# ChikaYan/mvs_gaussian_splatting

Hardware: AMD Instinct MI355X
Metric: Mpixels/s fwd + train-step ms @1080p, 6M Gaussians, 1->8 MI355X (higher is better)
Workload: dtype f32

## Files before the change

### mvs_gaussian_splatting_amd/csrc/gsr_api.hip

```cpp
#include <hip/hip_runtime.h>
#include <dlfcn.h>
#include <stdio.h>
#include <string.h>
#include <atomic>
#include <mutex>
#include <string>
#include <vector>

#include "gsr_common.h"
#include "gsr_launch.h"

using namespace gsr;

namespace {
thread_local std::string g_err = "";

int fail(int code, const char* msg) {
  g_err = msg;
  return code;
}
int hip_fail(hipError_t e, const char* where) {
  g_err = std::string(where) + ": " + hipGetErrorString(e);
  return (int)e;
}
// ... 157 lines not shown

size_t gsr_geom_bytes(int32_t P) { return GeomLayout(P < 0 ? 0 : P).bytes; }
size_t gsr_image_bytes(int32_t width, int32_t height) { return ImageLayout(width, height).bytes; }
size_t gsr_binning_bytes(uint32_t num_rendered, uint32_t num_visible, int32_t, int32_t, int32_t mode) {
  return BinLayout(num_rendered, num_visible, mode).bytes;
}
size_t gsr_backward_bytes(int32_t P, uint32_t num_rendered) { return BwdLayout(P, num_rendered).bytes; }
size_t gsr_camera_grad_bytes(int32_t P) { return camera_grad_bytes(P); }
size_t gsr_sort_scratch_bytes(uint32_t n) { return SortLayout(n).bytes; }

}

static void enqueue_depth_top_pass(const GsrParams* p, void* geom_ws, hipStream_t s);

enum TopPass { TOP_PASS_WITH, TOP_PASS_LATER, TOP_PASS_NEVER };
static int enqueue_stage1(const GsrParams* p, void* geom_ws, int32_t* radii, hipStream_t s, uint32_t capacity,
                          hipEvent_t counted, TopPass top_pass) {
  const GeomLayout L(p->P);
  {
    StageTimer t(p, GSR_STAGE_PREPROCESS_FWD, s);
    launch_preprocess_fwd(*p, at<GeomRec>(geom_ws, L.rec), at<BinInfo>(geom_ws, L.bin),
                          at<uint32_t>(geom_ws, L.block_sums), at<uint32_t>(geom_ws, L.block_vis), radii,
                          at<uint32_t>(geom_ws, L.block_big), at<uint32_t>(geom_ws, L.big_list),
                          at<uint2>(geom_ws, L.block_range), s);
  }
  if (int rc = check(p, s, "preprocess_fwd")) return rc;
  uint32_t* total = at<uint32_t>(geom_ws, L.total);
  {
    StageTimer t(p, GSR_STAGE_SCAN, s);
    launch_scan_block_sums(at<uint32_t>(geom_ws, L.block_sums), at<uint32_t>(geom_ws, L.block_offs), total + TOTAL_R,
                           at<uint32_t>(geom_ws, L.block_vis), at<uint32_t>(geom_ws, L.block_vis_offs), total + TOTAL_V,
                           L.nblocks, s, p->counts_pinned, at<uint2>(geom_ws, L.block_range),
                           at<uint32_t>(geom_ws, L.block_big), at<uint32_t>(geom_ws, L.block_big_offs), total + TOTAL_BIG);
  }
  if (int rc = check(p, s, "scan_block_sums")) return rc;
  if (counted) GSR_HIP(hipEventRecord(counted, s));
  if (p->binning_mode != GSR_BINNING_KEYS64) {
    StageTimer t(p, GSR_STAGE_SORT, s);
    launch_compact_visible(p->P, at<BinInfo>(geom_ws, L.bin), at<uint32_t>(geom_ws, L.block_vis_offs),
                           at<uint32_t>(geom_ws, L.block_offs),
                           p->forward_only ? nullptr : at<uint32_t>(geom_ws, L.slot_base), total, capacity,
                           (p->width + TILE - 1) / TILE, at<uint32_t>(geom_ws, L.dkey_a), at<uint2>(geom_ws, L.didx_a), s,
                           top_pass != TOP_PASS_NEVER);
    launch_sort_pairs_u32_v64(at<uint32_t>(geom_ws, L.dkey_a), at<uint2>(geom_ws, L.didx_a),
                              at<uint32_t>(geom_ws, L.dkey_b), at<uint2>(geom_ws, L.didx_b), (uint32_t)p->P,
                              DEPTH_SORT_BITS, at<char>(geom_ws, L.dsort), s, total + TOTAL_V);
    if (top_pass == TOP_PASS_WITH) enqueue_depth_top_pass(p, geom_ws, s);
// ... 274 lines not shown
  const ImageLayout I(p->width, p->height);
  GradRow* rows = at<GradRow>(bwd_ws, Wl.rows);
  uint8_t* flags = at<uint8_t>(bwd_ws, Wl.flags);
  const GeomRec* rec = at<GeomRec>(geom_ws, L.rec);
  if (R > 0) {
    if (!bin_ws) return fail(GSR_E_BADARG, "bin_ws is NULL");
    const SortedViews sv = sorted_views(bin_ws, R, V, p->width, p->height, p->binning_mode);
    const uint32_t* point_list = sv.point_list;
    GSR_HIP(hipMemsetAsync(flags, 0, R, s));
    {
      StageTimer t(p, GSR_STAGE_RENDER_BWD, s);
      launch_render_bwd(p->width, p->height, at<uint2>(img_ws, I.ranges), point_list, rec,
                        at<uint32_t>(geom_ws, L.slot_base), p->bg,
                        at<float>(img_ws, I.final_T), at<uint32_t>(img_ws, I.n_contrib),
                        at<uint32_t>(img_ws, I.tile_max), dL_dout_color, rows, flags,
                        at<uint32_t>(img_ws, I.tile_order), s, sv.inst_mask);
    }
    if (int rc = check(p, s, "render_bwd")) return rc;
  }
  {
    StageTimer t(p, GSR_STAGE_PREPROCESS_BWD, s);
    launch_sum_big_rows(at<uint32_t>(geom_ws, L.total) + TOTAL_BIG, at<uint32_t>(geom_ws, L.block_big_offs), L.nblocks,
                        at<uint32_t>(geom_ws, L.big_list), rec, at<uint32_t>(geom_ws, L.slot_base), rows, flags, s);
    launch_preprocess_bwd(*p, radii, rec, at<uint32_t>(geom_ws, L.slot_base), rows, flags, *grads, s);
  }
  return check(p, s, "preprocess_bwd");
}

int gsr_profile_create(void** handle) {
  if (!handle) return fail(GSR_E_BADARG, "handle is NULL");
  *handle = new Profile();
  return 0;
}
int gsr_profile_destroy(void* handle) {
  Profile* pr = static_cast<Profile*>(handle);
  if (!pr) return 0;
  for (auto& sp : pr->used) { if (sp.a) (void)hipEventDestroy(sp.a); if (sp.b) (void)hipEventDestroy(sp.b); }
  for (auto e : pr->pool) (void)hipEventDestroy(e);
  delete pr;
  return 0;
}
int gsr_profile_collect(void* handle, double* ms_sum, uint32_t* counts) {
  Profile* pr = static_cast<Profile*>(handle);
  if (!pr || !ms_sum || !counts) return fail(GSR_E_BADARG, "NULL argument");
  std::vector<Profile::Span> spans;
  {
    std::lock_guard<std::mutex> lock(pr->mu);
// ... 542 lines not shown
```

### mvs_gaussian_splatting_amd/csrc/gsr_common.h

```cpp
#pragma once
#include <hip/hip_runtime.h>
#include <stdint.h>
#include "../../include/gsr.h"

namespace gsr {

constexpr int TILE = 16;
constexpr int WAVE = 64;
constexpr float NEAR_Z = 0.2f;
constexpr float DILATION = 0.3f;
constexpr float FOV_GUARD = 1.3f;
constexpr float ALPHA_MAX = 0.99f;
constexpr float ALPHA_MIN = 1.0f / 255.0f;
constexpr float T_STOP = 0.0001f;

struct __attribute__((aligned(64))) GeomRec {
  float x, y, cxx, cxy;
  float cyy, opacity, r, g;
  float b, ext_x, ext_y;
  uint32_t tile_mask;
  uint32_t rect_min;
  uint32_t rect_wh;
  float kk;
  float isyy;
// ... 66 lines not shown
#ifndef GSR_SORT_ITEMS
#define GSR_SORT_ITEMS 8
#endif
constexpr int SORT_ITEMS = GSR_SORT_ITEMS;
constexpr int SORT_TILE = SORT_THREADS * SORT_ITEMS;
constexpr int RADIX_BITS = 9;
constexpr int RADIX = 1 << RADIX_BITS;

struct SortLayout {
  size_t hist, totals, totals_odd, bytes;
  uint32_t nblocks;
  __host__ __device__ explicit SortLayout(uint32_t n) {
    nblocks = (n + SORT_TILE - 1) / SORT_TILE;
    if (nblocks == 0) nblocks = 1;
    nblocks += RADIX;
    size_t o = 0;
    hist = o;   o = align_up(o + 4 * (size_t)RADIX * nblocks, 256);
    totals = o; o = align_up(o + 4 * (size_t)RADIX, 256);
    totals_odd = o; o = align_up(o + 4 * (size_t)RADIX, 256);
    bytes = o;
  }
};

struct GeomLayout {
  size_t rec, bin, offsets, slot_base, block_sums, block_offs, block_vis, block_vis_offs, block_range, total;
  size_t dkey_a, dkey_b, didx_a, didx_b, dsort, big_list, block_big, block_big_offs, bytes;
  int nblocks;
  __host__ __device__ explicit GeomLayout(int P) {
    nblocks = (P + PRE_BLOCK - 1) / PRE_BLOCK;
    size_t o = 0;
    rec = o;        o = align_up(o + sizeof(GeomRec) * (size_t)P, 256);
    bin = o;        o = align_up(o + sizeof(BinInfo) * (size_t)P, 256);
    offsets = o;    o = align_up(o + 4 * (size_t)P, 256);
    slot_base = o;  o = align_up(o + 4 * (size_t)P, 256);
    block_sums = o; o = align_up(o + 4 * (size_t)(nblocks + 1), 256);
    block_offs = o; o = align_up(o + 4 * (size_t)(nblocks + 1), 256);
    block_vis = o;  o = align_up(o + 4 * (size_t)(nblocks + 1), 256);
    block_vis_offs = o; o = align_up(o + 4 * (size_t)(nblocks + 1), 256);
    block_range = o; o = align_up(o + 8 * (size_t)(nblocks + 1), 256);
    total = o;      o = align_up(o + 64, 256);
    dkey_a = o;     o = align_up(o + 4 * (size_t)P, 256);
    dkey_b = o;     o = align_up(o + 4 * (size_t)P, 256);
    didx_a = o;     o = align_up(o + 8 * (size_t)P, 256);
    didx_b = o;     o = align_up(o + 8 * (size_t)P, 256);
    dsort = o;      o = align_up(o + SortLayout((uint32_t)(P > 0 ? P : 1)).bytes, 256);
    big_list = o;   o = align_up(o + 4 * (size_t)nblocks * PRE_BLOCK, 256);
    block_big = o;  o = align_up(o + 4 * (size_t)(nblocks + 1), 256);
    block_big_offs = o; o = align_up(o + 4 * (size_t)(nblocks + 1), 256);
    bytes = o;
  }
};

enum {
  TOTAL_R = 0,
  TOTAL_V = 1,
  TOTAL_BIG = 2,
  TOTAL_DEPTH_INV_MIN = 4,
  TOTAL_DEPTH_MAX = 5,
  TOTAL_TOP_PASS_N = 6,
  TOTAL_R_CLAMPED = 7
};
constexpr int DEPTH_SORT_BITS = 24;

struct ImageLayout {
  size_t final_T, n_contrib, ranges, tile_max, tile_order, bytes;
  int grid_x, grid_y, tiles;
  __host__ __device__ ImageLayout(int W, int H) {
    grid_x = (W + TILE - 1) / TILE;
    grid_y = (H + TILE - 1) / TILE;
    tiles = grid_x * grid_y;
    size_t o = 0;
// ... 99 lines not shown
```

### mvs_gaussian_splatting_amd/csrc/gsr_launch.h

```cpp
#pragma once
#include "gsr_common.h"

namespace gsr {

void launch_preprocess_fwd(const GsrParams& p, GeomRec* rec, BinInfo* bin, uint32_t* block_sums, uint32_t* block_vis,
                           int32_t* radii, uint32_t* block_big, uint32_t* big_list, uint2* block_range, hipStream_t s);
void launch_sum_big_rows(const uint32_t* big_count, const uint32_t* big_offs, int nb, const uint32_t* big_list,
                         const GeomRec* rec, const uint32_t* slot_base, GradRow* rows, uint8_t* row_flags, hipStream_t s);
void launch_scan_block_sums(const uint32_t* sums_a, uint32_t* offs_a, uint32_t* total_a, const uint32_t* sums_b,
                            uint32_t* offs_b, uint32_t* total_b, int nb, hipStream_t s,
                            uint32_t* host_mirror = nullptr, const uint2* block_range = nullptr,
                            const uint32_t* sums_c = nullptr, uint32_t* offs_c = nullptr, uint32_t* total_c = nullptr);
void launch_preprocess_bwd(const GsrParams& p, const int32_t* radii, const GeomRec* rec, const uint32_t* slot_base,
                           const GradRow* rows,
                           const uint8_t* row_flags, const GsrGrads& g, hipStream_t s);
size_t camera_grad_bytes(int P);
void launch_camera_grad_finish(const GsrGrads& g, int nslots, hipStream_t s);

void launch_duplicate_with_keys(int P, int grid_x, const BinInfo* bin, const uint32_t* block_offs, uint32_t* slot_base,
                                uint32_t* point_offsets, uint64_t* keys, uint32_t* vals, hipStream_t s);
bool launch_sort_pairs(uint64_t* keys_a, uint32_t* vals_a, uint64_t* keys_b, uint32_t* vals_b, uint32_t n,
                       int end_bit, void* scratch, hipStream_t s);
struct SortedRuns {
  uint2* runs_rel;
  uint32_t n_keys;
  bool valid;
  bool relative;
  const uint32_t* totals_last;
  int lo_bits, hi_bits;
};
bool launch_sort_pairs_u32(uint32_t* keys_a, uint32_t* vals_a, uint32_t* keys_b, uint32_t* vals_b, uint32_t n,
                           int end_bit, void* scratch, hipStream_t s, const uint32_t* n_dev = nullptr,
                           SortedRuns* runs = nullptr);
void launch_identify_tile_ranges_u32(uint32_t R, const uint32_t* tiles, uint2* ranges, hipStream_t s,
                                     const uint32_t* r_dev = nullptr);
inline int sort_passes(int end_bit) { return (end_bit + RADIX_BITS - 1) / RADIX_BITS; }
void launch_identify_tile_ranges(uint32_t R, const uint64_t* keys, uint2* ranges, hipStream_t s);
void launch_build_tile_order(int tiles, const uint2* ranges, uint32_t* order, hipStream_t s);
// ... 117 lines not shown
```

### mvs_gaussian_splatting_amd/csrc/preprocess.hip

```cpp
#include "gsr_common.h"
#include "gsr_launch.h"

namespace gsr {

constexpr float SH_C0 = 0.28209479177387814f;
constexpr float SH_C1 = 0.4886025119029199f;
constexpr float SH_C2_0 = 1.0925484305920792f;
constexpr float SH_C2_1 = -1.0925484305920792f;
constexpr float SH_C2_2 = 0.31539156525252005f;
constexpr float SH_C2_3 = -1.0925484305920792f;
constexpr float SH_C2_4 = 0.5462742152960396f;
constexpr float SH_C3_0 = -0.5900435899266435f;
constexpr float SH_C3_1 = 2.890611442640554f;
constexpr float SH_C3_2 = -0.4570457994644658f;
constexpr float SH_C3_3 = 0.3731763325901154f;
constexpr float SH_C3_4 = -0.4570457994644658f;
constexpr float SH_C3_5 = 1.445305721320277f;
constexpr float SH_C3_6 = -0.5900435899266435f;

struct Mat4 { float m[16]; };

__device__ inline void load_mat(const float* __restrict__ src, Mat4& d) {
#pragma unroll
  for (int i = 0; i < 16; ++i) d.m[i] = src[i];
}
// ... 56 lines not shown
#pragma unroll
  for (int ch = 0; ch < 3; ++ch) {
    float res = SH_C0 * sh(0, ch);
    if (deg > 0) {
      res = res - SH_C1 * y * sh(1, ch) + SH_C1 * z * sh(2, ch) - SH_C1 * x * sh(3, ch);
      if (deg > 1) {
        const float xx = x * x, yy = y * y, zz = z * z, xy = x * y, yz = y * z, xz = x * z;
        res = res + SH_C2_0 * xy * sh(4, ch) + SH_C2_1 * yz * sh(5, ch) +
              SH_C2_2 * (2.0f * zz - xx - yy) * sh(6, ch) + SH_C2_3 * xz * sh(7, ch) +
              SH_C2_4 * (xx - yy) * sh(8, ch);
        if (deg > 2) {
          res = res + SH_C3_0 * y * (3.0f * xx - yy) * sh(9, ch) + SH_C3_1 * xy * z * sh(10, ch) +
                SH_C3_2 * y * (4.0f * zz - xx - yy) * sh(11, ch) +
                SH_C3_3 * z * (2.0f * zz - 3.0f * xx - 3.0f * yy) * sh(12, ch) +
                SH_C3_4 * x * (4.0f * zz - xx - yy) * sh(13, ch) + SH_C3_5 * z * (xx - yy) * sh(14, ch) +
                SH_C3_6 * x * (xx - 3.0f * yy) * sh(15, ch);
        }
      }
    }
    out[ch] = res;
  }
}

struct Activated {
  float sc[3];
  float4 q;
  float qn;
  float op;
};
__device__ inline void load_scale_rot_raw(const GsrParams& p, int idx, Activated& a) {
  a.sc[0] = p.scales[3 * (size_t)idx];
  a.sc[1] = p.scales[3 * (size_t)idx + 1];
  a.sc[2] = p.scales[3 * (size_t)idx + 2];
  a.q = reinterpret_cast<const float4*>(p.rotations)[idx];
}
__device__ inline void activate_scale_rot(const GsrParams& p, Activated& a) {
  if (p.act_flags & GSR_ACT_SCALE_EXP) {
#pragma unroll
    for (int k = 0; k < 3; ++k) a.sc[k] = expf(a.sc[k]);
  }
  a.qn = 1.0f;
  if (p.act_flags & GSR_ACT_ROT_NORMALIZE) {
    a.qn = fmaxf(sqrtf(a.q.x * a.q.x + a.q.y * a.q.y + a.q.z * a.q.z + a.q.w * a.q.w), 1e-12f);
    a.q.x = a.q.x / a.qn; a.q.y = a.q.y / a.qn; a.q.z = a.q.z / a.qn; a.q.w = a.q.w / a.qn;
  }
}
// ... 41 lines not shown
      st[f] = v.x; st[f + 1] = v.y; st[f + 2] = v.z; st[f + 3] = v.w;
    } else {
      for (int e = 0; e < 4; ++e)
        if (f + e < nfl) st[f + e] = src[f + e];
    }
  }
}
__device__ inline void wave_store_rows45(float* __restrict__ base, int first, int rows_valid, const float* st,
                                         int lane) {
  float* __restrict__ dst = base + (size_t)first * REST_ROW;
  const int nfl = rows_valid * REST_ROW;
#pragma unroll
  for (int i = 0; i < 12; ++i) {
    const int f = (i * WAVE + lane) * 4;
    if (f + 3 < nfl) {
      *reinterpret_cast<float4*>(dst + f) = make_float4(st[f], st[f + 1], st[f + 2], st[f + 3]);
    } else {
      for (int e = 0; e < 4; ++e)
        if (f + e < nfl) dst[f + e] = st[f + e];
    }
  }
}

__global__ __launch_bounds__(PRE_BLOCK) void preprocess_fwd_kernel(GsrParams p, GeomRec* __restrict__ rec,
                                                                   BinInfo* __restrict__ bin,
                                                                   uint32_t* __restrict__ block_sums,
                                                                   uint32_t* __restrict__ block_vis,
                                                                   int32_t* __restrict__ radii,
                                                                   uint32_t* __restrict__ block_big,
                                                                   uint32_t* __restrict__ big_list,
                                                                   uint2* __restrict__ block_range) {
  __shared__ uint32_t wave_big[PRE_BLOCK / WAVE];
  __shared__ uint32_t wave_sums[PRE_BLOCK / WAVE];
  __shared__ uint32_t wave_vis[PRE_BLOCK / WAVE];
  __shared__ uint2 wave_range[PRE_BLOCK / WAVE];
  const int idx = blockIdx.x * PRE_BLOCK + threadIdx.x;
  const int lane = threadIdx.x & (WAVE - 1), wid = threadIdx.x / WAVE;
  const int W = p.width, H = p.height;
  const int grid_x = (W + TILE - 1) / TILE, grid_y = (H + TILE - 1) / TILE;
  uint32_t tiles = 0;
  int32_t radius = 0;
  BinInfo bi{0u, 0u, 0.0f, 0u};
  GeomRec g;
  bool vis = false;
  int rx0 = 0, ry0 = 0, rw = 0, rh = 0;
  float px = 0.f, py = 0.f, pz = 0.f;
  Proj pr;
  pr.a = pr.c = 1.0f;
  Activated act;
  float op_raw = 0.0f;
  const bool sh_regs = !p.colors_precomp && (p.shs_rest != nullptr || p.M == 16);
  bool sh_early = false;
  float shrow[48];

  if (idx < p.P) {
    Mat4 V, Mx;
    load_mat(p.viewmatrix, V);
    load_mat(p.projmatrix, Mx);
    px = p.means3D[3 * (size_t)idx + 0]; py = p.means3D[3 * (size_t)idx + 1]; pz = p.means3D[3 * (size_t)idx + 2];
    if (!p.cov3D_precomp) load_scale_rot_raw(p, idx, act);
    op_raw = p.opacities[idx];
    const float vx = V.m[0] * px + V.m[4] * py + V.m[8] * pz + V.m[12];
    const float vy = V.m[1] * px + V.m[5] * py + V.m[9] * pz + V.m[13];
    const float vz = V.m[2] * px + V.m[6] * py + V.m[10] * pz + V.m[14];
    if (vz > NEAR_Z) {
      const float hx = Mx.m[0] * px + Mx.m[4] * py + Mx.m[8] * pz + Mx.m[12];
      const float hy = Mx.m[1] * px + Mx.m[5] * py + Mx.m[9] * pz + Mx.m[13];
      const float hw = Mx.m[3] * px + Mx.m[7] * py + Mx.m[11] * pz + Mx.m[15];
      const float p_w = 1.0f / (hw + 0.0000001f);
      const float ndc_x = hx * p_w, ndc_y = hy * p_w;
      if (sh_regs && fabsf(ndc_x) < 1.0f && fabsf(ndc_y) < 1.0f) {
        sh_early = true;
        load_sh_row48(p, idx, shrow);
      }

      float cov[6];
      if (p.cov3D_precomp) {
#pragma unroll
        for (int k = 0; k < 6; ++k) cov[k] = p.cov3D_precomp[6 * (size_t)idx + k];
      } else {
        activate_scale_rot(p, act);
        cov3d_from_scale_rot(act.sc[0], act.sc[1], act.sc[2], p.scale_modifier, act.q.x, act.q.y, act.q.z, act.q.w, cov);
      }
      const float fx = (float)W / (2.0f * p.tan_fovx), fy = (float)H / (2.0f * p.tan_fovy);
      project_cov(V, vx, vy, vz, cov, fx, fy, FOV_GUARD * p.tan_fovx, FOV_GUARD * p.tan_fovy, pr);
      const float det = pr.a * pr.c - pr.b * pr.b;
      if (det != 0.0f) {
        const float det_inv = 1.0f / det;
        const float mid = 0.5f * (pr.a + pr.c);
        const float sq = sqrtf(fmaxf(0.1f, mid * mid - det));
        const float lam = fmaxf(mid + sq, mid - sq);
        const float rad = ceilf(3.0f * sqrtf(lam));
        const float mx = ((ndc_x + 1.0f) * (float)W - 1.0f) * 0.5f;
        const float my = ((ndc_y + 1.0f) * (float)H - 1.0f) * 0.5f;
// ... 14 lines not shown
            g.tile_mask = full_mask(tiles);
            g.rect_min = (uint32_t)x0 | ((uint32_t)y0 << 16);
            g.rect_wh = (uint32_t)(x1 - x0) | ((uint32_t)(y1 - y0) << 16);
            g.kk = -pr.b / pr.c;
            g.isyy = 1.0f / pr.c;
            bi.depth = vz;
          }
        }
      }
    }
  }

  if (vis) {
    float rgb[3];
    uint32_t flags = 0;
    if (p.colors_precomp) {
      rgb[0] = p.colors_precomp[3 * (size_t)idx];
      rgb[1] = p.colors_precomp[3 * (size_t)idx + 1];
      rgb[2] = p.colors_precomp[3 * (size_t)idx + 2];
    } else {
      const float dx = px - p.campos[0], dy = py - p.campos[1], dz = pz - p.campos[2];
      const float ln = sqrtf(dx * dx + dy * dy + dz * dz);
      const float ux = dx / ln, uy = dy / ln, uz = dz / ln;
      if (sh_regs) {
        if (!sh_early) load_sh_row48(p, idx, shrow);
        eval_sh(p.D, [&](int k, int ch) { return shrow[3 * k + ch]; }, ux, uy, uz, rgb);
      } else {
        const float* __restrict__ s = p.shs + (size_t)idx * p.M * 3;
        eval_sh(p.D, [&](int k, int ch) { return s[3 * k + ch]; }, ux, uy, uz, rgb);
      }
#pragma unroll
      for (int ch = 0; ch < 3; ++ch) {
        rgb[ch] = rgb[ch] + 0.5f;
        if (rgb[ch] < 0.0f) flags |= 1u << ch;
        rgb[ch] = fmaxf(rgb[ch], 0.0f);
      }
    }
    const float op = activate_opacity(p, op_raw);
    float ext_x = -1.0f, ext_y = -1.0f;
    if (op >= ALPHA_MIN) {
      const float t = 2.0f * logf(op * 255.0f) * 1.0001f + 1e-4f;
      ext_x = sqrtf(t * pr.a) * 1.0001f + 0.01f;
      ext_y = sqrtf(t * pr.c) * 1.0001f + 0.01f;
    }
    g.opacity = op; g.r = rgb[0]; g.g = rgb[1]; g.b = rgb[2];
    g.ext_x = ext_x; g.ext_y = ext_y;
    if (p.binning_mode == GSR_BINNING_TWO_LEVEL_CULLED) {
      const float inv = 1.0f / (float)TILE;
      int tx_lo = 0, tx_hi = -1, ty_lo = 0, ty_hi = -1;
      if (ext_x >= 0.0f) {
        tx_lo = max(0, (int)ceilf((g.x - ext_x - 15.0f) * inv) - rx0);
// ... 22 lines not shown
          m = (tx_hi >= tx_lo && ty_hi >= ty_lo) ? 1u : 0u;
        } else if (tx_hi >= tx_lo && ty_hi >= ty_lo) {
          const float t = 2.0f * __logf(255.0f * op) * 1.001f + 2e-3f;
          const float icxx = __builtin_amdgcn_rcpf(g.cxx), icyy = __builtin_amdgcn_rcpf(g.cyy);
          for (int ty = ty_lo; ty <= ty_hi; ++ty) {
            const float dy0 = (float)((ry0 + ty) * TILE) - g.y;
            for (int tx = tx_lo; tx <= tx_hi; ++tx) {
              const float dx0 = (float)((rx0 + tx) * TILE) - g.x;
              if (!(qmin_rect(g.cxx, g.cxy, g.cyy, icxx, icyy, dx0, dx0 + 15.0f, dy0, dy0 + 15.0f) > t))
                m |= 1u << (ty * rw + tx);
            }
          }
        }
        g.tile_mask = m;
        tiles = (uint32_t)__popc(m);
      }
    }
    bi.rect_min = g.rect_min; bi.rect_wh = g.rect_wh;
    bi.mask = g.tile_mask;
    g.rect_min |= flags << 29;
    rec[idx] = g;
  }
  if (idx < p.P) {
    radii[idx] = radius;
    bin[idx] = bi;
    if (p.visible_out) p.visible_out[idx] = radius > 0 ? 1 : 0;
  }

  uint32_t dinv = tiles != 0u ? ~__float_as_uint(bi.depth) : 0u, dmax = tiles != 0u ? __float_as_uint(bi.depth) : 0u;
#pragma unroll
  for (int d = WAVE / 2; d > 0; d >>= 1) {
    dinv = max(dinv, (uint32_t)__shfl_xor((int)dinv, d, WAVE));
    dmax = max(dmax, (uint32_t)__shfl_xor((int)dmax, d, WAVE));
  }

  const uint32_t ws = wave_reduce_add_u32(tiles);
  const uint32_t wv = (uint32_t)__popcll(__ballot(tiles != 0u));
  const bool big = tiles > ROWS_COOP;
  const unsigned long long big_lanes = __ballot(big);
  if (lane == 0) {
    wave_sums[wid] = ws; wave_vis[wid] = wv; wave_range[wid] = make_uint2(dinv, dmax);
    wave_big[wid] = (uint32_t)__popcll(big_lanes);
  }
  __syncthreads();
  if (big) {
    uint32_t k = (uint32_t)__popcll(big_lanes & ((1ull << lane) - 1ull));
// ... 104 lines not shown
    } else {
#pragma unroll
      for (int k = 0; k < PER; ++k) {
        if (lo + k < nb) block_offs[lo + k] = run;
        run += v[k];
      }
    }
    carry += all;
  }
  if (tid == 0) {
    block_offs[nb] = carry;
    *total = carry;
    if (host_mirror && blockIdx.x < 2) host_mirror[blockIdx.x] = carry;
  }
}

constexpr int CAM_TERMS = 27;
template <bool CAM>
__global__ __launch_bounds__(PRE_BLOCK) void preprocess_bwd_kernel(GsrParams p, const int32_t* __restrict__ radii,
                                                                   const GeomRec* __restrict__ rec,
                                                                   const uint32_t* __restrict__ slot_base,
                                                                   const GradRow* __restrict__ rows,
                                                                   const uint8_t* __restrict__ row_flags,
                                                                   GsrGrads g) {
  constexpr int SH_ROW = 49;
  __shared__ float sh_stage[PRE_BLOCK / WAVE][WAVE * SH_ROW];
  const int idx = blockIdx.x * PRE_BLOCK + threadIdx.x;
  const bool valid = idx < p.P;
  const int lane = threadIdx.x & (WAVE - 1), wid = threadIdx.x / WAVE;
  const int M = p.M;
  const bool split = p.shs_rest != nullptr;
  const bool sh_lds = p.shs != nullptr && M == 16 && g.dL_dshs != nullptr;
  float* my_row = &sh_stage[wid][lane * SH_ROW];
  float dmean[3] = {0.f, 0.f, 0.f};
  float dm2x = 0.f, dm2y = 0.f, dop = 0.f;
  float dcol[3] = {0.f, 0.f, 0.f};
  float dcov[6] = {0.f, 0.f, 0.f, 0.f, 0.f, 0.f};
  float dscale[3] = {0.f, 0.f, 0.f};
  float drot[4] = {0.f, 0.f, 0.f, 0.f};
  float cam[CAM ? CAM_TERMS : 1];
  if constexpr (CAM) {
#pragma unroll
    for (int k = 0; k < CAM_TERMS; ++k) cam[k] = 0.f;
  }
  const bool vis = valid && radii[idx] > 0;
  const int wave_first = blockIdx.x * PRE_BLOCK + wid * WAVE;
// ... 208 lines not shown
      for (int i = 0; i < 3; ++i) {
        dmean[i] += (Mx.m[4 * i + 0] * m_w - Mx.m[4 * i + 3] * mul1) * dm2x +
                    (Mx.m[4 * i + 1] * m_w - Mx.m[4 * i + 3] * mul2) * dm2y;
      }
      if constexpr (CAM) {
        const float pq[4] = {px, py, pz, 1.0f};
        const float dhw = mul1 * dm2x + mul2 * dm2y;
#pragma unroll
        for (int i = 0; i < 4; ++i) {
          cam[12 + 3 * i + 0] = pq[i] * m_w * dm2x;
          cam[12 + 3 * i + 1] = pq[i] * m_w * dm2y;
          cam[12 + 3 * i + 2] = -(pq[i] * dhw);
        }
      }
    }

    if (p.shs) {
      float dc[3];
#pragma unroll
      for (int ch = 0; ch < 3; ++ch) dc[ch] = ((rect_clamp_flags(r.rect_min) >> ch) & 1u) ? 0.0f : dcol[ch];
      const float dxr = px - p.campos[0], dyr = py - p.campos[1], dzr = pz - p.campos[2];
      const float ln = sqrtf(dxr * dxr + dyr * dyr + dzr * dzr);
      const float x = dxr / ln, y = dyr / ln, z = dzr / ln;
      const float* __restrict__ s = p.shs + (size_t)idx * M * 3;
      float* __restrict__ ds = g.dL_dshs + (size_t)idx * M * 3;
      const int deg = p.D;
      float dRx[3] = {0.f, 0.f, 0.f}, dRy[3] = {0.f, 0.f, 0.f}, dRz[3] = {0.f, 0.f, 0.f};
      float4 sv4[12];
      if (M == 16 && !split) {
        const float4* s4 = reinterpret_cast<const float4*>(s);
#pragma unroll
        for (int k = 0; k < 12; ++k) sv4[k] = s4[k];
      } else if (split && deg > 0) {
        const float* __restrict__ rr = p.shs_rest + (size_t)idx * REST_ROW;
        float* f = reinterpret_cast<float*>(sv4);
#pragma unroll
        for (int i = 0; i < REST_ROW; ++i) f[3 + i] = rr[i];
      }
      const float* sreg = reinterpret_cast<const float*>(sv4);
      auto emit = [&](int k, float basis) {
#pragma unroll
        for (int ch = 0; ch < 3; ++ch) {
          const float v = basis * dc[ch];
          if (split) {
            if (k == 0) g.dL_dshs[3 * (size_t)idx + ch] = v;
            else my_row[3 * (k - 1) + ch] = v;
          } else if (sh_lds) {
            my_row[3 * k + ch] = v;
          } else {
            ds[3 * k + ch] = v;
          }
        }
      };
      auto dirg = [&](int k, float bx, float by, float bz) {
#pragma clang fp contract(fast)
#pragma unroll
        for (int ch = 0; ch < 3; ++ch) {
          const float c = (M == 16) ? sreg[3 * k + ch] : s[3 * k + ch];
          if (!(__builtin_constant_p(bx) && bx == 0.0f)) dRx[ch] += bx * c;
          if (!(__builtin_constant_p(by) && by == 0.0f)) dRy[ch] += by * c;
          if (!(__builtin_constant_p(bz) && bz == 0.0f)) dRz[ch] += bz * c;
        }
      };
      emit(0, SH_C0);
      if (deg > 0) {
        dirg(1, 0.f, -SH_C1, 0.f); dirg(2, 0.f, 0.f, SH_C1); dirg(3, -SH_C1, 0.f, 0.f);
        emit(1, -SH_C1 * y); emit(2, SH_C1 * z); emit(3, -SH_C1 * x);
        if (deg > 1) {
          const float xx = x * x, yy = y * y, zz = z * z, xy = x * y, yz = y * z, xz = x * z;
          dirg(4, SH_C2_0 * y, SH_C2_0 * x, 0.f);
          dirg(5, 0.f, SH_C2_1 * z, SH_C2_1 * y);
          dirg(6, SH_C2_2 * -2.0f * x, SH_C2_2 * -2.0f * y, SH_C2_2 * 4.0f * z);
          dirg(7, SH_C2_3 * z, 0.f, SH_C2_3 * x);
          dirg(8, SH_C2_4 * 2.0f * x, SH_C2_4 * -2.0f * y, 0.f);
          emit(4, SH_C2_0 * xy); emit(5, SH_C2_1 * yz); emit(6, SH_C2_2 * (2.0f * zz - xx - yy));
          emit(7, SH_C2_3 * xz); emit(8, SH_C2_4 * (xx - yy));
          if (deg > 2) {
            dirg(9, SH_C3_0 * 6.0f * xy, SH_C3_0 * (3.0f * xx - 3.0f * yy), 0.f);
            dirg(10, SH_C3_1 * yz, SH_C3_1 * xz, SH_C3_1 * xy);
            dirg(11, SH_C3_2 * -2.0f * xy, SH_C3_2 * (4.0f * zz - xx - 3.0f * yy), SH_C3_2 * 8.0f * yz);
            dirg(12, SH_C3_3 * -6.0f * xz, SH_C3_3 * -6.0f * yz, SH_C3_3 * (6.0f * zz - 3.0f * xx - 3.0f * yy));
            dirg(13, SH_C3_4 * (4.0f * zz - 3.0f * xx - yy), SH_C3_4 * -2.0f * xy, SH_C3_4 * 8.0f * xz);
            dirg(14, SH_C3_5 * 2.0f * xz, SH_C3_5 * -2.0f * yz, SH_C3_5 * (xx - yy));
            dirg(15, SH_C3_6 * (3.0f * xx - 3.0f * yy), SH_C3_6 * -6.0f * xy, 0.f);
            emit(9, SH_C3_0 * y * (3.0f * xx - yy)); emit(10, SH_C3_1 * xy * z);
            emit(11, SH_C3_2 * y * (4.0f * zz - xx - yy));
            emit(12, SH_C3_3 * z * (2.0f * zz - 3.0f * xx - 3.0f * yy));
            emit(13, SH_C3_4 * x * (4.0f * zz - xx - yy)); emit(14, SH_C3_5 * z * (xx - yy));
            emit(15, SH_C3_6 * x * (xx - 3.0f * yy));
          }
        }
      }
      const int used = (deg + 1) * (deg + 1);
      for (int k = used; k < M; ++k) emit(k, 0.0f);
      const float ddx = dRx[0] * dc[0] + dRx[1] * dc[1] + dRx[2] * dc[2];
      const float ddy = dRy[0] * dc[0] + dRy[1] * dc[1] + dRy[2] * dc[2];
      const float ddz = dRz[0] * dc[0] + dRz[1] * dc[1] + dRz[2] * dc[2];
      const float sum2 = dxr * dxr + dyr * dyr + dzr * dzr;
      const float inv3 = 1.0f / (ln * sum2);
      const float dd0 = ((sum2 - dxr * dxr) * ddx - dyr * dxr * ddy - dzr * dxr * ddz) * inv3;
      const float dd1 = (-dxr * dyr * ddx + (sum2 - dyr * dyr) * ddy - dzr * dyr * ddz) * inv3;
      const float dd2 = (-dxr * dzr * ddx - dyr * dzr * ddy + (sum2 - dzr * dzr) * ddz) * inv3;
      dmean[0] += dd0;
      dmean[1] += dd1;
      dmean[2] += dd2;
      if constexpr (CAM) {
        cam[24] = -dd0; cam[25] = -dd1; cam[26] = -dd2;
// ... 101 lines not shown
    g.stats_denom[idx] += 1.0f;
    g.stats_max_radii2D[idx] = fmaxf(g.stats_max_radii2D[idx], (float)radii[idx]);
  }
  if (g.dL_dcolors) {
#pragma unroll
    for (int i = 0; i < 3; ++i) g.dL_dcolors[3 * (size_t)idx + i] = dcol[i];
  }
  if (p.cov3D_precomp) {
    if (g.dL_dcov3D)
#pragma unroll
      for (int i = 0; i < 6; ++i) g.dL_dcov3D[6 * (size_t)idx + i] = dcov[i];
  } else {
    if (g.dL_dscales)
#pragma unroll
      for (int i = 0; i < 3; ++i) g.dL_dscales[3 * (size_t)idx + i] = dscale[i];
    if (g.dL_drotations)
#pragma unroll
      for (int i = 0; i < 4; ++i) g.dL_drotations[4 * (size_t)idx + i] = drot[i];
  }
}


void launch_preprocess_fwd(const GsrParams& p, GeomRec* rec, BinInfo* bin, uint32_t* block_sums, uint32_t* block_vis,
                           int32_t* radii, uint32_t* block_big, uint32_t* big_list, uint2* block_range, hipStream_t s) {
  const int nb = (p.P + PRE_BLOCK - 1) / PRE_BLOCK;
  if (nb > 0)
    hipLaunchKernelGGL(preprocess_fwd_kernel, dim3(nb), dim3(PRE_BLOCK), 0, s, p, rec, bin, block_sums, block_vis, radii,
                       block_big, big_list, block_range);
}
void launch_scan_block_sums(const uint32_t* sums_a, uint32_t* offs_a, uint32_t* total_a, const uint32_t* sums_b,
                            uint32_t* offs_b, uint32_t* total_b, int nb, hipStream_t s, uint32_t* host_mirror,
                            const uint2* block_range, const uint32_t* sums_c, uint32_t* offs_c, uint32_t* total_c) {
  hipLaunchKernelGGL(scan_block_sums_kernel, dim3(block_range ? (sums_c ? 4 : 3) : (sums_b ? 2 : 1)), dim3(1024), 0, s, sums_a,
                     offs_a, total_a, sums_b, offs_b, total_b, nb, host_mirror, block_range, sums_c, offs_c, total_c);
}
__global__ __launch_bounds__(256) void sum_big_rows_kernel(const uint32_t* __restrict__ big_count,
                                                           const uint32_t* __restrict__ big_offs, int nb,
                                                           const uint32_t* __restrict__ big_list,
                                                           const GeomRec* __restrict__ rec,
                                                           const uint32_t* __restrict__ slot_base,
                                                           GradRow* __restrict__ rows, uint8_t* __restrict__ row_flags) {
  const uint32_t count = *big_count;
  const int lane = threadIdx.x & (WAVE - 1);
  const uint32_t wave = blockIdx.x * (256 / WAVE) + threadIdx.x / WAVE, nwaves = gridDim.x * (256 / WAVE);
  const uint32_t per = (count + nwaves - 1) / nwaves;
  const uint32_t e0 = wave * per, e1 = min(count, e0 + per);
  if (e0 >= e1) return;
  int lo = 0, hi = nb - 1;
  while (lo < hi) {
    const int span = hi - lo, step = (span + WAVE - 1) / WAVE;
    const int pos = lo + (lane + 1) * step;
// ... 67 lines not shown
    for (int b = stripe; b < nslots; b += CAM_STRIPES) acc += slots[(size_t)b * CAM_TERMS + term];
    part[stripe][term] = acc;
  }
  __syncthreads();
  if (threadIdx.x < CAM_TERMS) {
    double acc = part[0][threadIdx.x];
    for (int k = 1; k < CAM_STRIPES; ++k) acc += part[k][threadIdx.x];
    tot[threadIdx.x] = acc;
  }
  __syncthreads();
  if (threadIdx.x < 16) {
    const int i = threadIdx.x >> 2, c = threadIdx.x & 3;
    dV[threadIdx.x] = c < 3 ? (float)tot[3 * i + c] : 0.0f;
    dM[threadIdx.x] = c == 2 ? 0.0f : (float)tot[12 + 3 * i + (c == 3 ? 2 : c)];
  }
  if (threadIdx.x < 3) dC[threadIdx.x] = (float)tot[24 + threadIdx.x];
}

size_t camera_grad_bytes(int P) {
  const size_t nb = P > 0 ? ((size_t)P + PRE_BLOCK - 1) / PRE_BLOCK : 0;
  return align_up((nb ? nb : 1) * CAM_TERMS * sizeof(double), 256);
}
void launch_preprocess_bwd(const GsrParams& p, const int32_t* radii, const GeomRec* rec, const uint32_t* slot_base,
                           const GradRow* rows, const uint8_t* row_flags, const GsrGrads& g, hipStream_t s) {
  const int nb = (p.P + PRE_BLOCK - 1) / PRE_BLOCK;
  if (!g.dL_dviewmatrix) {
    if (nb > 0) hipLaunchKernelGGL(preprocess_bwd_kernel<false>, dim3(nb), dim3(PRE_BLOCK), 0, s, p, radii, rec, slot_base, rows, row_flags, g);
    return;
  }
  if (nb > 0) hipLaunchKernelGGL(preprocess_bwd_kernel<true>, dim3(nb), dim3(PRE_BLOCK), 0, s, p, radii, rec, slot_base, rows, row_flags, g);
  launch_camera_grad_finish(g, nb, s);
}
void launch_camera_grad_finish(const GsrGrads& g, int nslots, hipStream_t s) {
  hipLaunchKernelGGL(camera_grad_finish_kernel, dim3(1), dim3(CAM_FINISH_THREADS), 0, s,
                     static_cast<const double*>(g.camera_ws), nslots, g.dL_dviewmatrix, g.dL_dprojmatrix, g.dL_dcampos);
}

}
```

Baseline: 2323.

## Precompute SH direction Jacobian in forward preprocess and reuse in backward

In training mode, the forward preprocess kernel now computes the spherical-harmonics direction Jacobian (9 floats per Gaussian) while the SH coefficients are already in registers, and stores it in SoA planes in the geometry workspace. The backward preprocess kernel reads these 9 values instead of reloading the 48 SH coefficients and recomputing the directional gradient. The goal is to cut backward memory traffic and ALU work. In exchange it adds forward stores and workspace memory, disables the early SH load in the training variant, and sets a waves-per-EU hint that may affect occupancy.

```diff
diff --git a/mvs_gaussian_splatting_amd/csrc/gsr_api.hip b/mvs_gaussian_splatting_amd/csrc/gsr_api.hip
--- a/mvs_gaussian_splatting_amd/csrc/gsr_api.hip
+++ b/mvs_gaussian_splatting_amd/csrc/gsr_api.hip
@@ -203,7 +203,7 @@
     launch_preprocess_fwd(*p, at<GeomRec>(geom_ws, L.rec), at<BinInfo>(geom_ws, L.bin),
                           at<uint32_t>(geom_ws, L.block_sums), at<uint32_t>(geom_ws, L.block_vis), radii,
                           at<uint32_t>(geom_ws, L.block_big), at<uint32_t>(geom_ws, L.big_list),
-                          at<uint2>(geom_ws, L.block_range), s);
+                          at<uint2>(geom_ws, L.block_range), at<float>(geom_ws, L.sh_jac), L.sh_jac_plane, s);
   }
   if (int rc = check(p, s, "preprocess_fwd")) return rc;
   uint32_t* total = at<uint32_t>(geom_ws, L.total);
@@ -524,7 +524,8 @@
     StageTimer t(p, GSR_STAGE_PREPROCESS_BWD, s);
     launch_sum_big_rows(at<uint32_t>(geom_ws, L.total) + TOTAL_BIG, at<uint32_t>(geom_ws, L.block_big_offs), L.nblocks,
                         at<uint32_t>(geom_ws, L.big_list), rec, at<uint32_t>(geom_ws, L.slot_base), rows, flags, s);
-    launch_preprocess_bwd(*p, radii, rec, at<uint32_t>(geom_ws, L.slot_base), rows, flags, *grads, s);
+    launch_preprocess_bwd(*p, radii, rec, at<uint32_t>(geom_ws, L.slot_base), rows, flags, at<float>(geom_ws, L.sh_jac),
+                          L.sh_jac_plane, *grads, s);
   }
   return check(p, s, "preprocess_bwd");
 }
diff --git a/mvs_gaussian_splatting_amd/csrc/gsr_common.h b/mvs_gaussian_splatting_amd/csrc/gsr_common.h
--- a/mvs_gaussian_splatting_amd/csrc/gsr_common.h
+++ b/mvs_gaussian_splatting_amd/csrc/gsr_common.h
@@ -112,9 +112,11 @@
   }
 };
 
+constexpr int SH_JAC_PLANES = 9;
 struct GeomLayout {
   size_t rec, bin, offsets, slot_base, block_sums, block_offs, block_vis, block_vis_offs, block_range, total;
-  size_t dkey_a, dkey_b, didx_a, didx_b, dsort, big_list, block_big, block_big_offs, bytes;
+  size_t dkey_a, dkey_b, didx_a, didx_b, dsort, big_list, block_big, block_big_offs;
+  size_t sh_jac, sh_jac_plane, bytes;
   int nblocks;
   __host__ __device__ explicit GeomLayout(int P) {
     nblocks = (P + PRE_BLOCK - 1) / PRE_BLOCK;
@@ -137,6 +139,13 @@
     big_list = o;   o = align_up(o + 4 * (size_t)nblocks * PRE_BLOCK, 256);
     block_big = o;  o = align_up(o + 4 * (size_t)(nblocks + 1), 256);
     block_big_offs = o; o = align_up(o + 4 * (size_t)(nblocks + 1), 256);
+#ifdef EXP_ROWS4
+    sh_jac_plane = align_up(16 * (size_t)P, 256) / 4;
+    sh_jac = o;     o = o + 3 * 4 * sh_jac_plane;
+#else
+    sh_jac_plane = align_up(4 * (size_t)P, 256) / 4;
+    sh_jac = o;     o = o + SH_JAC_PLANES * 4 * sh_jac_plane;
+#endif
     bytes = o;
   }
 };
diff --git a/mvs_gaussian_splatting_amd/csrc/gsr_launch.h b/mvs_gaussian_splatting_amd/csrc/gsr_launch.h
--- a/mvs_gaussian_splatting_amd/csrc/gsr_launch.h
+++ b/mvs_gaussian_splatting_amd/csrc/gsr_launch.h
@@ -4,7 +4,8 @@
 namespace gsr {
 
 void launch_preprocess_fwd(const GsrParams& p, GeomRec* rec, BinInfo* bin, uint32_t* block_sums, uint32_t* block_vis,
-                           int32_t* radii, uint32_t* block_big, uint32_t* big_list, uint2* block_range, hipStream_t s);
+                           int32_t* radii, uint32_t* block_big, uint32_t* big_list, uint2* block_range, float* sh_jac,
+                           size_t jac_plane, hipStream_t s);
 void launch_sum_big_rows(const uint32_t* big_count, const uint32_t* big_offs, int nb, const uint32_t* big_list,
                          const GeomRec* rec, const uint32_t* slot_base, GradRow* rows, uint8_t* row_flags, hipStream_t s);
 void launch_scan_block_sums(const uint32_t* sums_a, uint32_t* offs_a, uint32_t* total_a, const uint32_t* sums_b,
@@ -12,8 +13,8 @@
                             uint32_t* host_mirror = nullptr, const uint2* block_range = nullptr,
                             const uint32_t* sums_c = nullptr, uint32_t* offs_c = nullptr, uint32_t* total_c = nullptr);
 void launch_preprocess_bwd(const GsrParams& p, const int32_t* radii, const GeomRec* rec, const uint32_t* slot_base,
-                           const GradRow* rows,
-                           const uint8_t* row_flags, const GsrGrads& g, hipStream_t s);
+                           const GradRow* rows, const uint8_t* row_flags, const float* sh_jac, size_t jac_plane,
+                           const GsrGrads& g, hipStream_t s);
 size_t camera_grad_bytes(int P);
 void launch_camera_grad_finish(const GsrGrads& g, int nslots, hipStream_t s);
 
diff --git a/mvs_gaussian_splatting_amd/csrc/preprocess.hip b/mvs_gaussian_splatting_amd/csrc/preprocess.hip
--- a/mvs_gaussian_splatting_amd/csrc/preprocess.hip
+++ b/mvs_gaussian_splatting_amd/csrc/preprocess.hip
@@ -1,6 +1,12 @@
 #include "gsr_common.h"
 #include "gsr_launch.h"
 
+#ifndef EXP_WAVES
+#define EXP_WAVES 4
+#endif
+#ifndef EXP_EARLY
+#define EXP_EARLY 0
+#endif
 namespace gsr {
 
 constexpr float SH_C0 = 0.28209479177387814f;
@@ -103,6 +109,45 @@
   }
 }
 
+template <typename LoadSH>
+__device__ inline void sh_dir_jacobian(int deg, LoadSH sh, float x, float y, float z, float* dRx, float* dRy, float* dRz) {
+  auto dirg = [&](int k, float bx, float by, float bz) {
+#pragma clang fp contract(fast)
+#pragma unroll
+    for (int ch = 0; ch < 3; ++ch) {
+      const float c = sh(k, ch);
+      if (!(__builtin_constant_p(bx) && bx == 0.0f)) dRx[ch] += bx * c;
+      if (!(__builtin_constant_p(by) && by == 0.0f)) dRy[ch] += by * c;
+      if (!(__builtin_constant_p(bz) && bz == 0.0f)) dRz[ch] += bz * c;
+    }
+#ifndef EXP_NO_SB
+    __builtin_amdgcn_sched_barrier(0);
+#endif
+  };
+#pragma unroll
+  for (int ch = 0; ch < 3; ++ch) dRx[ch] = dRy[ch] = dRz[ch] = 0.f;
+  if (deg > 0) {
+    dirg(1, 0.f, -SH_C1, 0.f); dirg(2, 0.f, 0.f, SH_C1); dirg(3, -SH_C1, 0.f, 0.f);
+    if (deg > 1) {
+      const float xx = x * x, yy = y * y, zz = z * z, xy = x * y, yz = y * z, xz = x * z;
+      dirg(4, SH_C2_0 * y, SH_C2_0 * x, 0.f);
+      dirg(5, 0.f, SH_C2_1 * z, SH_C2_1 * y);
+      dirg(6, SH_C2_2 * -2.0f * x, SH_C2_2 * -2.0f * y, SH_C2_2 * 4.0f * z);
+      dirg(7, SH_C2_3 * z, 0.f, SH_C2_3 * x);
+      dirg(8, SH_C2_4 * 2.0f * x, SH_C2_4 * -2.0f * y, 0.f);
+      if (deg > 2) {
+        dirg(9, SH_C3_0 * 6.0f * xy, SH_C3_0 * (3.0f * xx - 3.0f * yy), 0.f);
+        dirg(10, SH_C3_1 * yz, SH_C3_1 * xz, SH_C3_1 * xy);
+        dirg(11, SH_C3_2 * -2.0f * xy, SH_C3_2 * (4.0f * zz - xx - 3.0f * yy), SH_C3_2 * 8.0f * yz);
+        dirg(12, SH_C3_3 * -6.0f * xz, SH_C3_3 * -6.0f * yz, SH_C3_3 * (6.0f * zz - 3.0f * xx - 3.0f * yy));
+        dirg(13, SH_C3_4 * (4.0f * zz - 3.0f * xx - yy), SH_C3_4 * -2.0f * xy, SH_C3_4 * 8.0f * xz);
+        dirg(14, SH_C3_5 * 2.0f * xz, SH_C3_5 * -2.0f * yz, SH_C3_5 * (xx - yy));
+        dirg(15, SH_C3_6 * (3.0f * xx - 3.0f * yy), SH_C3_6 * -6.0f * xy, 0.f);
+      }
+    }
+  }
+}
+
 struct Activated {
   float sc[3];
   float4 q;
@@ -190,14 +235,16 @@
   }
 }
 
-__global__ __launch_bounds__(PRE_BLOCK) void preprocess_fwd_kernel(GsrParams p, GeomRec* __restrict__ rec,
+template <bool SAVE_JAC>
+__global__ __launch_bounds__(PRE_BLOCK) __attribute__((amdgpu_waves_per_eu(SAVE_JAC ? EXP_WAVES : 1))) void preprocess_fwd_kernel(GsrParams p, GeomRec* __restrict__ rec,
                                                                    BinInfo* __restrict__ bin,
                                                                    uint32_t* __restrict__ block_sums,
                                                                    uint32_t* __restrict__ block_vis,
                                                                    int32_t* __restrict__ radii,
                                                                    uint32_t* __restrict__ block_big,
                                                                    uint32_t* __restrict__ big_list,
-                                                                   uint2* __restrict__ block_range) {
+                                                                   uint2* __restrict__ block_range,
+                                                                   float* __restrict__ sh_jac, size_t jac_plane) {
   __shared__ uint32_t wave_big[PRE_BLOCK / WAVE];
   __shared__ uint32_t wave_sums[PRE_BLOCK / WAVE];
   __shared__ uint32_t wave_vis[PRE_BLOCK / WAVE];
@@ -237,7 +284,7 @@
       const float hw = Mx.m[3] * px + Mx.m[7] * py + Mx.m[11] * pz + Mx.m[15];
       const float p_w = 1.0f / (hw + 0.0000001f);
       const float ndc_x = hx * p_w, ndc_y = hy * p_w;
-      if (sh_regs && fabsf(ndc_x) < 1.0f && fabsf(ndc_y) < 1.0f) {
+      if ((!SAVE_JAC || EXP_EARLY) && sh_regs && fabsf(ndc_x) < 1.0f && fabsf(ndc_y) < 1.0f) {
         sh_early = true;
         load_sh_row48(p, idx, shrow);
       }
@@ -298,11 +345,28 @@
       const float dx = px - p.campos[0], dy = py - p.campos[1], dz = pz - p.campos[2];
       const float ln = sqrtf(dx * dx + dy * dy + dz * dz);
       const float ux = dx / ln, uy = dy / ln, uz = dz / ln;
+      auto save_jac = [&](auto sh) {
+        if (p.D > 0) {
+          float jac[SH_JAC_PLANES];
+          sh_dir_jacobian(p.D, sh, ux, uy, uz, jac, jac + 3, jac + 6);
+#ifdef EXP_ROWS4
+#pragma unroll
+          for (int k = 0; k < 3; ++k)
+            reinterpret_cast<float4*>(sh_jac + (size_t)k * jac_plane)[idx] = make_float4(jac[3 * k], jac[3 * k + 1], jac[3 * k + 2], 0.0f);
+#else
+#pragma unroll
+          for (int k = 0; k < SH_JAC_PLANES; ++k) sh_jac[(size_t)k * jac_plane + (size_t)idx] = jac[k];
+#endif
+        }
+        __builtin_amdgcn_sched_barrier(0);
+      };
       if (sh_regs) {
         if (!sh_early) load_sh_row48(p, idx, shrow);
+        if constexpr (SAVE_JAC) save_jac([&](int k, int ch) { return shrow[3 * k + ch]; });
         eval_sh(p.D, [&](int k, int ch) { return shrow[3 * k + ch]; }, ux, uy, uz, rgb);
       } else {
         const float* __restrict__ s = p.shs + (size_t)idx * p.M * 3;
+        if constexpr (SAVE_JAC) save_jac([&](int k, int ch) { return s[3 * k + ch]; });
         eval_sh(p.D, [&](int k, int ch) { return s[3 * k + ch]; }, ux, uy, uz, rgb);
       }
 #pragma unroll
@@ -371,6 +435,19 @@
     rec[idx] = g;
   }
   if (idx < p.P) {
+    if constexpr (SAVE_JAC) {
+#ifndef EXP_NO_FILL
+      if (!vis && p.shs && p.D > 0) {
+#ifdef EXP_ROWS4
+#pragma unroll
+        for (int k = 0; k < 3; ++k) reinterpret_cast<float4*>(sh_jac + (size_t)k * jac_plane)[idx] = make_float4(0.f, 0.f, 0.f, 0.f);
+#else
+#pragma unroll
+        for (int k = 0; k < SH_JAC_PLANES; ++k) sh_jac[(size_t)k * jac_plane + (size_t)idx] = 0.0f;
+#endif
+      }
+#endif
+    }
     radii[idx] = radius;
     bin[idx] = bi;
     if (p.visible_out) p.visible_out[idx] = radius > 0 ? 1 : 0;
@@ -521,6 +598,7 @@
                                                                    const uint32_t* __restrict__ slot_base,
                                                                    const GradRow* __restrict__ rows,
                                                                    const uint8_t* __restrict__ row_flags,
+                                                                   const float* __restrict__ sh_jac, size_t jac_plane,
                                                                    GsrGrads g) {
   constexpr int SH_ROW = 49;
   __shared__ float sh_stage[PRE_BLOCK / WAVE][WAVE * SH_ROW];
@@ -775,22 +853,27 @@
       const float dxr = px - p.campos[0], dyr = py - p.campos[1], dzr = pz - p.campos[2];
       const float ln = sqrtf(dxr * dxr + dyr * dyr + dzr * dzr);
       const float x = dxr / ln, y = dyr / ln, z = dzr / ln;
-      const float* __restrict__ s = p.shs + (size_t)idx * M * 3;
       float* __restrict__ ds = g.dL_dshs + (size_t)idx * M * 3;
       const int deg = p.D;
       float dRx[3] = {0.f, 0.f, 0.f}, dRy[3] = {0.f, 0.f, 0.f}, dRz[3] = {0.f, 0.f, 0.f};
-      float4 sv4[12];
-      if (M == 16 && !split) {
-        const float4* s4 = reinterpret_cast<const float4*>(s);
-#pragma unroll
-        for (int k = 0; k < 12; ++k) sv4[k] = s4[k];
-      } else if (split && deg > 0) {
-        const float* __restrict__ rr = p.shs_rest + (size_t)idx * REST_ROW;
-        float* f = reinterpret_cast<float*>(sv4);
-#pragma unroll
-        for (int i = 0; i < REST_ROW; ++i) f[3 + i] = rr[i];
-      }
-      const float* sreg = reinterpret_cast<const float*>(sv4);
+      if (deg > 0) {
+#ifdef EXP_ROWS4
+        const float4 jx = reinterpret_cast<const float4*>(sh_jac)[idx];
+        const float4 jy = reinterpret_cast<const float4*>(sh_jac + jac_plane)[idx];
+        const float4 jz = reinterpret_cast<const float4*>(sh_jac + 2 * jac_plane)[idx];
+        dRx[0] = jx.x; dRx[1] = jx.y; dRx[2] = jx.z;
+        dRy[0] = jy.x; dRy[1] = jy.y; dRy[2] = jy.z;
+        dRz[0] = jz.x; dRz[1] = jz.y; dRz[2] = jz.z;
+#else
+        const float* __restrict__ j = sh_jac + (size_t)idx;
+#pragma unroll
+        for (int ch = 0; ch < 3; ++ch) {
+          dRx[ch] = j[(size_t)ch * jac_plane];
+          dRy[ch] = j[(size_t)(3 + ch) * jac_plane];
+          dRz[ch] = j[(size_t)(6 + ch) * jac_plane];
+        }
+#endif
+      }
       auto emit = [&](int k, float basis) {
 #pragma unroll
         for (int ch = 0; ch < 3; ++ch) {
@@ -805,37 +888,14 @@
           }
         }
       };
-      auto dirg = [&](int k, float bx, float by, float bz) {
-#pragma clang fp contract(fast)
-#pragma unroll
-        for (int ch = 0; ch < 3; ++ch) {
-          const float c = (M == 16) ? sreg[3 * k + ch] : s[3 * k + ch];
-          if (!(__builtin_constant_p(bx) && bx == 0.0f)) dRx[ch] += bx * c;
-          if (!(__builtin_constant_p(by) && by == 0.0f)) dRy[ch] += by * c;
-          if (!(__builtin_constant_p(bz) && bz == 0.0f)) dRz[ch] += bz * c;
-        }
-      };
       emit(0, SH_C0);
       if (deg > 0) {
-        dirg(1, 0.f, -SH_C1, 0.f); dirg(2, 0.f, 0.f, SH_C1); dirg(3, -SH_C1, 0.f, 0.f);
         emit(1, -SH_C1 * y); emit(2, SH_C1 * z); emit(3, -SH_C1 * x);
         if (deg > 1) {
           const float xx = x * x, yy = y * y, zz = z * z, xy = x * y, yz = y * z, xz = x * z;
-          dirg(4, SH_C2_0 * y, SH_C2_0 * x, 0.f);
-          dirg(5, 0.f, SH_C2_1 * z, SH_C2_1 * y);
-          dirg(6, SH_C2_2 * -2.0f * x, SH_C2_2 * -2.0f * y, SH_C2_2 * 4.0f * z);
-          dirg(7, SH_C2_3 * z, 0.f, SH_C2_3 * x);
-          dirg(8, SH_C2_4 * 2.0f * x, SH_C2_4 * -2.0f * y, 0.f);
           emit(4, SH_C2_0 * xy); emit(5, SH_C2_1 * yz); emit(6, SH_C2_2 * (2.0f * zz - xx - yy));
           emit(7, SH_C2_3 * xz); emit(8, SH_C2_4 * (xx - yy));
           if (deg > 2) {
-            dirg(9, SH_C3_0 * 6.0f * xy, SH_C3_0 * (3.0f * xx - 3.0f * yy), 0.f);
-            dirg(10, SH_C3_1 * yz, SH_C3_1 * xz, SH_C3_1 * xy);
-            dirg(11, SH_C3_2 * -2.0f * xy, SH_C3_2 * (4.0f * zz - xx - 3.0f * yy), SH_C3_2 * 8.0f * yz);
-            dirg(12, SH_C3_3 * -6.0f * xz, SH_C3_3 * -6.0f * yz, SH_C3_3 * (6.0f * zz - 3.0f * xx - 3.0f * yy));
-            dirg(13, SH_C3_4 * (4.0f * zz - 3.0f * xx - yy), SH_C3_4 * -2.0f * xy, SH_C3_4 * 8.0f * xz);
-            dirg(14, SH_C3_5 * 2.0f * xz, SH_C3_5 * -2.0f * yz, SH_C3_5 * (xx - yy));
-            dirg(15, SH_C3_6 * (3.0f * xx - 3.0f * yy), SH_C3_6 * -6.0f * xy, 0.f);
             emit(9, SH_C3_0 * y * (3.0f * xx - yy)); emit(10, SH_C3_1 * xy * z);
             emit(11, SH_C3_2 * y * (4.0f * zz - xx - yy));
             emit(12, SH_C3_3 * z * (2.0f * zz - 3.0f * xx - 3.0f * yy));
@@ -983,11 +1043,16 @@
 
 
 void launch_preprocess_fwd(const GsrParams& p, GeomRec* rec, BinInfo* bin, uint32_t* block_sums, uint32_t* block_vis,
-                           int32_t* radii, uint32_t* block_big, uint32_t* big_list, uint2* block_range, hipStream_t s) {
+                           int32_t* radii, uint32_t* block_big, uint32_t* big_list, uint2* block_range, float* sh_jac,
+                           size_t jac_plane, hipStream_t s) {
   const int nb = (p.P + PRE_BLOCK - 1) / PRE_BLOCK;
-  if (nb > 0)
-    hipLaunchKernelGGL(preprocess_fwd_kernel, dim3(nb), dim3(PRE_BLOCK), 0, s, p, rec, bin, block_sums, block_vis, radii,
-                       block_big, big_list, block_range);
+  if (nb <= 0) return;
+  if (p.forward_only)
+    hipLaunchKernelGGL(preprocess_fwd_kernel<false>, dim3(nb), dim3(PRE_BLOCK), 0, s, p, rec, bin, block_sums, block_vis, radii,
+                       block_big, big_list, block_range, sh_jac, jac_plane);
+  else
+    hipLaunchKernelGGL(preprocess_fwd_kernel<true>, dim3(nb), dim3(PRE_BLOCK), 0, s, p, rec, bin, block_sums, block_vis, radii,
+                       block_big, big_list, block_range, sh_jac, jac_plane);
 }
 void launch_scan_block_sums(const uint32_t* sums_a, uint32_t* offs_a, uint32_t* total_a, const uint32_t* sums_b,
                             uint32_t* offs_b, uint32_t* total_b, int nb, hipStream_t s, uint32_t* host_mirror,
@@ -1101,13 +1166,14 @@
   return align_up((nb ? nb : 1) * CAM_TERMS * sizeof(double), 256);
 }
 void launch_preprocess_bwd(const GsrParams& p, const int32_t* radii, const GeomRec* rec, const uint32_t* slot_base,
-                           const GradRow* rows, const uint8_t* row_flags, const GsrGrads& g, hipStream_t s) {
+                           const GradRow* rows, const uint8_t* row_flags, const float* sh_jac, size_t jac_plane,
+                           const GsrGrads& g, hipStream_t s) {
   const int nb = (p.P + PRE_BLOCK - 1) / PRE_BLOCK;
   if (!g.dL_dviewmatrix) {
-    if (nb > 0) hipLaunchKernelGGL(preprocess_bwd_kernel<false>, dim3(nb), dim3(PRE_BLOCK), 0, s, p, radii, rec, slot_base, rows, row_flags, g);
+    if (nb > 0) hipLaunchKernelGGL(preprocess_bwd_kernel<false>, dim3(nb), dim3(PRE_BLOCK), 0, s, p, radii, rec, slot_base, rows, row_flags, sh_jac, jac_plane, g);
     return;
   }
-  if (nb > 0) hipLaunchKernelGGL(preprocess_bwd_kernel<true>, dim3(nb), dim3(PRE_BLOCK), 0, s, p, radii, rec, slot_base, rows, row_flags, g);
+  if (nb > 0) hipLaunchKernelGGL(preprocess_bwd_kernel<true>, dim3(nb), dim3(PRE_BLOCK), 0, s, p, radii, rec, slot_base, rows, row_flags, sh_jac, jac_plane, g);
   launch_camera_grad_finish(g, nb, s);
 }
 void launch_camera_grad_finish(const GsrGrads& g, int nslots, hipStream_t s) {
```

Measured after the change: 2317. About the same (-0.3%).
